# livesense-inc/fanlin-rs

Hardware: AMD Instinct MI355X
Metric: images/sec whole-node (1080p→300×200 resize+encode); p50 per-image ms (higher is better)
Workload: dtype u8 (exact, as f16 subnormals) x the reference's f32 weights as three f16 terms -> f32 sums (vertical, v_mfma_f32_16x16x32_f16); 24-bit fixed-point intermediate (2^-14 steps, three i8 planes) x 24-bit fixed-point weights (2^-24 steps, three i8 digits), eight of the nine digit products -> exact i32 (h

## Files before the change

fanlin-rs_amd/csrc/fl_batch.cpp:

```cpp
#include <stdio.h>
#include <stdlib.h>

#include <algorithm>
#include <cassert>
#include <memory>
#include <optional>

#include "fl_context.h"

using namespace fl;

namespace {


enum Stage1Kind { S1_NONE = 0, S1_PLACE = 1, S1_GENERIC = 2, S1_STREAM = 3, S1_NEAREST = 4, S1_MFMA = 5, S1_TILE = 6, S1_WTILE = 7 };
constexpr size_t kNoScratch = ~(size_t)0;

struct Work {
    flgpu_plan plan;
    const flgpu_params *p;
    uint32_t cs, pre, sw, sh;
    Stage1Kind s1;
    const uint8_t *src;
    uint8_t *s1_dst = nullptr;
// ... 156 lines not shown
                        const auto &v = by_job[jobs_in_order[r * T + t]];
                        for (uint32_t s2 = 0; s2 < S; ++s2) per_wg[triples[t][s2]].push_back(v[s2]);
                    }
                const uint32_t Lp = P - R * T;
                if (Lp) {
                    const uint32_t nt = (uint32_t)plan->tiles.size();
                    const uint32_t nb = std::max(1u, std::min(nt, (2u * G + Lp * S - 1u) / (Lp * S)));
                    const std::vector<MfmaItem> &bands = plan->items_for(nb);
                    std::vector<MfmaItem> units;
                    for (uint32_t p2 = R * T; p2 < P; ++p2)
                        for (MfmaItem u : bands) { u.job = jobs_in_order[p2]; units.push_back(u); }
                    std::stable_sort(units.begin(), units.end(), [](const MfmaItem &x, const MfmaItem &y) { return x.kb1 - x.kb0 > y.kb1 - y.kb0; });
                    std::vector<uint64_t> load(G, 0);
                    for (uint32_t b = 0; b < G; ++b) for (const MfmaItem &a : per_wg[b]) load[b] += a.kb1 - a.kb0;
                    for (const MfmaItem &u : units) {
                        uint32_t best = 0;
                        for (uint32_t b = 1; b < G; ++b) if (load[b] < load[best]) best = b;
                        per_wg[best].push_back(u);
                        load[best] += u.kb1 - u.kb0 + 2u;
                    }
                }
            }
        }
    }
    if (!uniform) { for (auto &v : per_wg) v.clear(); classic(); }
    std::vector<MfmaItem> flat;
    lists.assign(2u * G, 0u);
    for (uint32_t b = 0; b < G; ++b) {
        lists[2 * b] = (uint32_t)flat.size();
        lists[2 * b + 1] = (uint32_t)per_wg[b].size();
        flat.insert(flat.end(), per_wg[b].begin(), per_wg[b].end());
    }
    mitems.resize(base);
    mitems.insert(mitems.end(), flat.begin(), flat.end());
    nitems = (uint32_t)flat.size();
}

void fill_job(const Work &w, Job &j)
{
    memset(&j, 0, sizeof(j));
    const flgpu_plan &pl = w.plan;
    j.src = w.src;
    j.dst = w.s1_dst;
    j.src_bytes = w.sw * w.sh * w.cs;
    j.sw = w.sw; j.sh = w.sh;
    j.rw = pl.resized_w; j.rh = pl.resized_h;
    j.cx = pl.crop_x; j.cy = pl.crop_y;
    if (pl.letterboxed) {
        j.cw = std::min(pl.resized_w - pl.crop_x, pl.out_w - pl.place_x);
        j.ch = std::min(pl.resized_h - pl.crop_y, pl.out_h - pl.place_y);
    } else {
        j.cw = pl.out_w; j.ch = pl.out_h;
    }
    j.dw = pl.out_w; j.dh = pl.out_h;
    j.ox = pl.place_x; j.oy = pl.place_y;
    if (w.luma_mid) { j.dw = j.cw; j.dh = j.ch; j.ox = 0; j.oy = 0; }
    j.fill = (uint32_t)w.p->fill_r | ((uint32_t)w.p->fill_g << 8) | ((uint32_t)w.p->fill_b << 16) | (255u << 24);
    j.vtab = w.vtab; j.htab = w.htab;
    j.pad1 = w.tile_w;
    j.pad0 = w.tile_vplan;
    if (w.s1 == S1_NEAREST) {
        const float ry = (float)w.sh / (float)pl.resized_h, rx = (float)w.sw / (float)pl.resized_w;
        memcpy(&j.vtab, &ry, 4); memcpy(&j.htab, &rx, 4);
    }
}


uint32_t tile_width_for(const HostAxis &h, const HostAxis &v, uint32_t cx, uint32_t cw, uint32_t cy, uint32_t ch, uint32_t mc)
{
    for (uint32_t y0 = cy; y0 < cy + ch; y0 += 8u) {
        const uint32_t y1 = std::min(y0 + 8u, cy + ch);
        if (v.left[y1 - 1] + v.count[y1 - 1] - v.left[y0] > kTileVRows) return 0;
    }
    const uint32_t nc_max = kTileLdsFloats / (8u * mc);
    for (uint32_t tw = 256; tw >= 16; tw >>= 1) {
        bool fits = true;
        for (uint32_t x0 = cx; x0 < cx + cw && fits; x0 += tw) {
            const uint32_t x1 = std::min(x0 + tw, cx + cw);
            if (h.left[x1 - 1] + h.count[x1 - 1] - h.left[x0] > nc_max) fits = false;
            if (h.woff[x1 - 1] + h.count[x1 - 1] - h.woff[x0] > kTileWeightFloats) fits = false;
        }
        if (fits) return tw;
    }
    return 0;
}

void build_tile_vplan(const HostAxis &v, uint32_t cy, uint32_t ch, std::vector<uint32_t> &blk)
{
    const uint32_t nb = (ch + 7u) / 8u;
    uint32_t stride = 1;
    for (uint32_t b = 0; b < nb; ++b) {
        const uint32_t y0 = cy + 8u * b, y1 = std::min(y0 + 8u, cy + ch);
        stride = std::max(stride, v.left[y1 - 1] + v.count[y1 - 1] - v.left[y0]);
    }
    TileVPlanHeader hd{nb, stride, (uint32_t)(sizeof(TileVPlanHeader) / 4), (uint32_t)(sizeof(TileVPlanHeader) / 4) + 2u * nb};
    blk.assign((size_t)hd.dense_off + (size_t)nb * stride * 8u, 0u);
    memcpy(blk.data(), &hd, sizeof(hd));
    for (uint32_t b = 0; b < nb; ++b) {
        const uint32_t y0 = cy + 8u * b, y1 = std::min(y0 + 8u, cy + ch);
        const uint32_t top = v.left[y0], rv = v.left[y1 - 1] + v.count[y1 - 1] - top;
        blk[hd.bands_off + 2u * b] = top;
        blk[hd.bands_off + 2u * b + 1u] = rv;
        float *dense = reinterpret_cast<float *>(blk.data() + hd.dense_off) + (size_t)b * stride * 8u;
        for (uint32_t oy = y0; oy < y1; ++oy)
            for (uint32_t k = 0; k < v.count[oy]; ++k) dense[(size_t)(v.left[oy] + k - top) * 8u + (oy - y0)] = v.weights[v.woff[oy] + k];
    }
}

template <class Item, class Len>
void xcd_interleave(Item *first, uint32_t nitems, Len len_of)
{
#ifdef FL_EXPERIMENT
    static const bool no_xcd_order = [] { const char *e = getenv("FLGPU_NO_XCD_ORDER"); return e && e[0] == '1'; }();
#else
    constexpr bool no_xcd_order = false;
#endif
    std::vector<Item> tmp;
    for (uint32_t a = 0; a < nitems && !no_xcd_order;) {
        uint32_t b = a;
        const uint32_t len = len_of(first[a]);
        while (b < nitems && len_of(first[b]) == len) ++b;
        for (uint32_t g0 = a; g0 < b;) {
            uint32_t g1 = g0, njob = 0, prev = 0xffffffffu, per = 0, cur = 0;
            bool uniform = true;
            while (g1 < b) {
                if (first[g1].job != prev) {
                    if (njob == 8) break;
                    if (njob >= 1) { if (per == 0) per = cur; else if (cur != per) uniform = false; }
                    ++njob; prev = first[g1].job; cur = 0;
                }
                ++cur; ++g1;
            }
            if (per == 0) per = cur; else if (cur != per) uniform = false;
            if (uniform && njob > 1 && per > 1) {
                tmp.assign(first + g0, first + g1);
                for (uint32_t s2 = 0; s2 < per; ++s2)
                    for (uint32_t j2 = 0; j2 < njob; ++j2) first[g0 + s2 * njob + j2] = tmp[j2 * per + s2];
            }
            g0 = g1;
        }
        a = b;
    }
}



int jpeg_scratch(const flgpu_plan &pl, ScratchSizes &s)
{
    if (pl.out_w > 65535u || pl.out_h > 65535u) return FLGPU_ERR_UNSUPPORTED;
    const size_t units = (size_t)(pl.plane_w / 8u) * (pl.plane_h / 8u) * 3u;
    if (units * kJpegMaxUnitBytes * 8 >= ((size_t)1 << 32)) return FLGPU_ERR_UNSUPPORTED;
    s.jpeg_coef += align_up(units * sizeof(uint32_t), 256);
    s.jpeg_off += align_up((units + 1) * sizeof(uint32_t), 256);
    s.jpeg_raw += align_up(units * kAcWordsPerUnit * sizeof(uint32_t), 256);
    return FLGPU_OK;
}

int png_scratch(const flgpu_plan &pl, ScratchSizes &s)
{
    const uint64_t fb = png_filtered_bytes(pl.out_w, pl.out_h, pl.out_c);
    if ((uint64_t)s.png_rows + pl.out_h >= (1ull << 31) || (uint64_t)s.png_segs + png_segments(fb) >= (1ull << 31)) return FLGPU_ERR_UNSUPPORTED;
    s.png_filt += align_up(fb, 256);
    s.png_rows += pl.out_h;
    s.png_segs += (uint32_t)png_segments(fb);
    return FLGPU_OK;
}

int webpll_scratch(const flgpu_plan &pl, ScratchSizes &s)
{
    const uint64_t npix = (uint64_t)pl.out_w * pl.out_h;
    if ((uint64_t)s.wll_tiles + webpll_tiles(npix) >= (1ull << 31) || webpll_max_out_bytes(pl.out_w, pl.out_h) / 4u >= (1ull << 32))
        return FLGPU_ERR_UNSUPPORTED;
    s.wll_res += align_up(npix * 4u, 256);
    s.wll_tok += align_up(npix * 2u, 256);
    s.wll_stream += align_up(webpll_max_out_bytes(pl.out_w, pl.out_h), 256);
    s.wll_tiles += (uint32_t)webpll_tiles(npix);
    s.wll_pics++;
    return FLGPU_OK;
}

int plan_pictures(Batch &B, const flgpu_image *srcs, const flgpu_params *ps, bool same_params)
{
    for (size_t i = 0; i < B.n; ++i) {
        Work &w = B.work[i];
        const flgpu_image &s = srcs[i];
        w.p = same_params ? &ps[0] : &ps[i];
        if (!s.data || !B.dsts[i].data) return FLGPU_ERR_INVALID_ARG;
        int rc = flgpu_plan_output(w.p, s.width, s.height, s.channels, &w.plan);
        if (rc) return rc;
        if (s.capacity < (uint64_t)s.width * s.height * s.channels) return FLGPU_ERR_INVALID_ARG;
        if (B.dsts[i].capacity < w.plan.out_bytes) return FLGPU_ERR_BUFFER_TOO_SMALL;
        w.cs = s.channels; w.sw = w.plan.src_w; w.sh = w.plan.src_h;
        w.raw_w = s.width; w.raw_h = s.height;
        w.orient = w.p->orientation >= 2 ? w.p->orientation : 0;
        if (w.orient) { w.orient_off = B.scratch.o; B.scratch.o += align_up((size_t)s.width * s.height * s.channels, 256); }
        w.pre = w.p->grayscale ? PRE_GRAY : (w.p->inverse ? PRE_INVERT : PRE_NONE);
        w.src = s.data;
        w.final_dst = B.dsts[i].data;
        const flgpu_plan &pl = w.plan;
        const bool cropped = pl.crop_x || pl.crop_y || pl.out_w != pl.resized_w || pl.out_h != pl.resized_h;
        const bool pre_changes = (w.pre == PRE_INVERT) || (w.pre == PRE_GRAY && w.cs >= 3);
        if (!pre_changes) w.pre = PRE_NONE;
        if (pl.resampled) w.s1 = w.p->filter == FLGPU_FILTER_NEAREST ? S1_NEAREST : S1_GENERIC;
        else if (pre_changes || pl.letterboxed || cropped) w.s1 = S1_PLACE;
        else w.s1 = S1_NONE;
        const bool mfma_candidate = !B.dbg.on(DBG_NO_MFMA) && !B.dbg.on(DBG_FORCE_GENERIC) && (size_t)w.sw * w.cs >= 64u && (uint64_t)w.sh >= 2u * (uint64_t)pl.resized_h;
        if (pl.resampled && w.s1 == S1_GENERIC && !pre_changes && !w.orient && mfma_candidate && ((size_t)w.sw * w.cs) % 16u == 0 && (uintptr_t)s.data % 16u != 0) {
            w.align_off = B.scratch.al;
            B.scratch.al += align_up((size_t)s.width * s.height * s.channels, 256);
        }
        const bool blur = w.p->blur_sigma > 0.0f;
        const bool fe = w.p->front_end != FLGPU_FE_NONE;
        if (w.s1 != S1_NONE && !blur && !fe) w.s1_dst = w.final_dst;
        else if (w.s1 != S1_NONE) { w.s1_off = B.scratch.a; B.scratch.a += align_up(pl.pixel_bytes, 256); }
        if (blur && !fe) w.blur_dst = w.final_dst;
        else if (blur) { w.blur_off = B.scratch.b; B.scratch.b += align_up(pl.pixel_bytes, 256); }
        if (w.p->front_end == FLGPU_FE_JPEG) rc = jpeg_scratch(pl, B.scratch);
        if (w.p->front_end == FLGPU_FE_PNG) rc = png_scratch(pl, B.scratch);
        if (w.p->front_end == FLGPU_FE_WEBP_LOSSLESS) rc = webpll_scratch(pl, B.scratch);
        if (rc) return rc;
    }
    return FLGPU_OK;
}

int reserve_scratch(flgpu_ctx *c, Batch &B, hipStream_t st)
{
    const ScratchSizes &sz = B.scratch;
    FL_HIP(c, c->d_jpeg_coef.reserve(sz.jpeg_coef), "JPEG coefficient scratch");
    FL_HIP(c, c->d_jpeg_off.reserve(sz.jpeg_off), "JPEG offset scratch");
    FL_HIP(c, c->d_jpeg_raw.reserve(sz.jpeg_raw), "JPEG bit-stream scratch");
    FL_HIP(c, c->d_png_filt.reserve(sz.png_filt), "PNG filtered-row scratch");
    FL_HIP(c, c->d_png_chunks.reserve((size_t)sz.png_segs * kPngSegOutBytes), "PNG chunk scratch");
    FL_HIP(c, c->d_png_syms.reserve((size_t)sz.png_segs * kPngSegBytes * sizeof(uint16_t)), "PNG symbol scratch");
    FL_HIP(c, c->d_png_recs.reserve((size_t)sz.png_segs * 4u * sizeof(uint32_t)), "PNG segment records");
    FL_HIP(c, c->d_webpll_res.reserve(sz.wll_res), "WebP residual scratch");
    FL_HIP(c, c->d_webpll_tok.reserve(sz.wll_tok), "WebP token scratch");
    FL_HIP(c, c->d_webpll_tiles.reserve((size_t)sz.wll_tiles * sizeof(WebpllTile)), "WebP tile records");
    FL_HIP(c, c->d_webpll_pic.reserve((size_t)sz.wll_pics * kWebpllPicWords * sizeof(uint32_t)), "WebP per-picture scratch");
    FL_HIP(c, c->d_webpll_stream.reserve(sz.wll_stream), "WebP bit-stream scratch");
    FL_HIP(c, c->d_tmp_o.reserve(sz.o), "orientation scratch");
    FL_HIP(c, c->d_tmp_al.reserve(sz.al), "alignment scratch");
    for (auto &w : B.work)
        if (w.align_off != kNoScratch) {
            uint8_t *al = static_cast<uint8_t *>(c->d_tmp_al.p) + w.align_off;
            FL_HIP(c, hipMemcpyAsync(al, w.src, (size_t)w.sw * w.sh * w.cs, hipMemcpyDeviceToDevice, st), "alignment copy");
            w.src = al;
        }
    FL_HIP(c, c->d_tmp_a.reserve(sz.a), "scratch A");
    FL_HIP(c, c->d_tmp_b.reserve(sz.b), "scratch B");
    for (auto &w : B.work) {
        if (w.orient) { w.raw_src = w.src; w.src = static_cast<uint8_t *>(c->d_tmp_o.p) + w.orient_off; }
        if (w.s1 == S1_NONE) w.s1_dst = const_cast<uint8_t *>(w.src);
        if (w.s1_off != kNoScratch) w.s1_dst = static_cast<uint8_t *>(c->d_tmp_a.p) + w.s1_off;
        if (w.blur_off != kNoScratch) w.blur_dst = static_cast<uint8_t *>(c->d_tmp_b.p) + w.blur_off;
    }
    return FLGPU_OK;
}


bool arena_nearly_full(const flgpu_ctx *c) { return c->h_arena.size() >= c->arena_cap_words - 1024; }

template <class Map, class Build> uint32_t cached_block(flgpu_ctx *c, Map &cache, const typename Map::key_type &key, Build &&build)
{
    auto it = cache.find(key);
    if (it != cache.end()) return it->second;
    std::vector<uint32_t> blk;
    build(blk);
    const uint32_t off = arena_append(c, blk.data(), blk.size());
    if (off) cache.emplace(key, off);
    return off;
}

bool try_wtile(flgpu_ctx *c, Work &w, const Job &j)
{
    WtPlan *wp = get_wtile_plan(c, w.vk, *w.va, w.hk, *w.ha, j.cx, j.cy, j.cw, j.ch, w.cs);
    if (wp->arena_full || arena_nearly_full(c)) return false;
    if (wp->ok) { w.s1 = S1_WTILE; w.wplan = wp; }
    return true;
}

bool try_mfma(flgpu_ctx *c, const DebugSwitches &dbg, size_t n_resample, Work &w, const Job &j)
{
    MfmaPlan *mp = get_mfma_plan(c, w.vk, *w.va, w.hk, *w.ha, j.cx, j.cy, j.cw, j.ch, w.cs, dbg.on(DBG_MFMA_ARITH) ? MFMA_ARITH_PACKED : MFMA_ARITH_FULL);
    if (mp->arena_full || arena_nearly_full(c)) return false;
    if (!mp->ok) return true;
    uint32_t nbands = (uint32_t)std::max<int64_t>(0, dbg.get(DBG_FORCE_BANDS));
    if (!nbands && n_resample < 128) {
        const uint64_t G = std::max(1u, c->cu_count);
        uint64_t best = ~0ull;
        for (uint32_t b = 1; b <= std::min<uint32_t>(16u, (uint32_t)mp->tiles.size()); ++b) {
            const std::vector<MfmaItem> &cand = mp->items_for(b);
            uint32_t longest = 0;
            for (const MfmaItem &mi : cand) longest = std::max(longest, mi.kb1 - mi.kb0);
            const uint64_t cost = (((uint64_t)n_resample * cand.size() + G - 1) / G) * (longest + 2u);
            if (cost < best) { best = cost; nbands = b; }
        }
    }
    w.s1 = S1_MFMA; w.mplan = mp; w.mitems = &mp->items_for(std::max(nbands, 1u));
    return true;
}

bool try_stream(flgpu_ctx *c, const DebugSwitches &dbg, size_t n_resample, Work &w, const Job &j)
{
    uint32_t nbands = (uint32_t)std::max<int64_t>(0, dbg.get(DBG_FORCE_BANDS));
    if (!nbands && n_resample < 512) nbands = std::min((uint32_t)((1024 + n_resample * 2 - 1) / (n_resample * 2)), j.ch / 24u);
    nbands = std::min(std::max(nbands, 1u), std::max(1u, j.ch));
    const StreamPlan *sp = get_stream_plan(c, w.vk, *w.va, w.hk, *w.ha, j.cx, j.cy, j.cw, j.ch, nbands, w.cs, w.pre);
// ... 984 lines not shown
```

fanlin-rs_amd/csrc/fl_jpeg.h:

```cpp
#pragma once
#include <hip/hip_runtime.h>
#include <stdint.h>

namespace fl {

#define FL_JPEG_RESULT_OVERFLOW 4u
constexpr uint32_t kAcWordsPerUnit = 52;
struct alignas(16) JpegJob {
    const uint8_t *src;
    uint8_t *dst;
    uint32_t *meta;
    uint32_t *unit_off;
    uint32_t *acbits;
    uint32_t *result;
    uint32_t w, h, c;
    uint32_t bx, by;
    uint32_t tab_off;
    uint32_t pad0;
    uint32_t dst_cap;
};

hipError_t launch_jpeg_encode(const JpegJob *jobs, const uint32_t *arena, uint32_t job_base, uint32_t njobs, uint32_t max_blocks,
                              hipStream_t st);

}
```

fanlin-rs_amd/csrc/fl_jpeg.hip:

```cpp
#include <hip/hip_runtime.h>
#include <stdint.h>

#include "fl_jpeg.h"
#include "fl_jpeg_tables.h"
#include "fl_pixel.h"
#include "fl_types.h"

namespace fl {

namespace {


constexpr int32_t F_0_298 = 2446, F_0_390 = 3196, F_0_541 = 4433, F_0_765 = 6270, F_0_899 = 7373, F_1_175 = 9633, F_1_501 = 12299,
                  F_1_847 = 15137, F_1_961 = 16069, F_2_053 = 16819, F_2_562 = 20995, F_3_072 = 25172;

struct Mat8 { int32_t a[8][8]; };

constexpr void fdct_linear(const int32_t in[8], int32_t out[8])
{
    int32_t t0 = in[0] + in[7], t1 = in[1] + in[6], t2 = in[2] + in[5], t3 = in[3] + in[4];
    const int32_t t10 = t0 + t3, t11 = t1 + t2;
    int32_t t12 = t0 - t3, t13 = t1 - t2;
    t0 = in[0] - in[7]; t1 = in[1] - in[6]; t2 = in[2] - in[5]; t3 = in[3] - in[4];
    out[0] = t10 + t11;
    out[4] = t10 - t11;
    int32_t z1 = (t12 + t13) * F_0_541;
    out[2] = z1 + t12 * F_0_765;
    out[6] = z1 - t13 * F_1_847;
    t12 = t0 + t2;
    t13 = t1 + t3;
    z1 = (t12 + t13) * F_1_175;
    t12 = t12 * (-F_0_390) + z1;
    t13 = t13 * (-F_1_961) + z1;
    z1 = (t0 + t3) * (-F_0_899);
    out[1] = t0 * F_1_501 + z1 + t12;
    out[7] = t3 * F_0_298 + z1 + t13;
    z1 = (t1 + t2) * (-F_2_562);
    out[3] = t1 * F_3_072 + z1 + t13;
    out[5] = t2 * F_2_053 + z1 + t12;
}

constexpr Mat8 make_fdct_matrix()
{
    Mat8 m{};
    for (int j = 0; j < 8; ++j) {
        int32_t e[8] = {0, 0, 0, 0, 0, 0, 0, 0}, o[8] = {0, 0, 0, 0, 0, 0, 0, 0};
        e[j] = 1;
        fdct_linear(e, o);
        for (int k = 0; k < 8; ++k) m.a[k][j] = o[k];
    }
    return m;
}

__constant__ Mat8 kFdct = make_fdct_matrix();

constexpr bool fdct_matrix_fits_i16()
{
    const Mat8 m = make_fdct_matrix();
    for (int k = 0; k < 8; ++k)
        for (int j = 0; j < 8; ++j)
            if (m.a[k][j] > 32767 || m.a[k][j] < -32768) return false;
    return true;
}
static_assert(fdct_matrix_fits_i16(), "the passes use v_dot2_i32_i16: matrix entries must be 16-bit");

typedef short i16x2 __attribute__((ext_vector_type(2)));
__device__ __forceinline__ i16x2 as_i16x2(uint32_t v) { return __builtin_bit_cast(i16x2, v); }
__device__ __forceinline__ uint32_t pack_i16(int32_t lo, int32_t hi) { return ((uint32_t)lo & 0xffffu) | ((uint32_t)hi << 16); }
__device__ __forceinline__ int32_t dot8_i16(const uint32_t m[4], const uint4 v)
{
    int32_t p = __builtin_amdgcn_sdot2(as_i16x2(m[0]), as_i16x2(v.x), 0, false);
    p = __builtin_amdgcn_sdot2(as_i16x2(m[1]), as_i16x2(v.y), p, false);
    p = __builtin_amdgcn_sdot2(as_i16x2(m[2]), as_i16x2(v.z), p, false);
    return __builtin_amdgcn_sdot2(as_i16x2(m[3]), as_i16x2(v.w), p, false);
}

struct NaturalOrder { uint8_t n[64]; };
constexpr NaturalOrder make_natural()
{
    NaturalOrder t{};
    for (int k = 0; k < 64; ++k) t.n[k] = kUnzigzag[k];
    return t;
}
__constant__ NaturalOrder kNatural = make_natural();

struct HuffLut { uint32_t e[256]; };

constexpr HuffLut make_lut(const HuffSpec &s)
{
    HuffLut t{};
    uint32_t code = 0;
    int k = 0;
    for (int l = 1; l <= 16; ++l) {
        for (int i = 0; i < s.len[l - 1]; ++i, ++k) t.e[s.val[k]] = ((uint32_t)l << 16) | code++;
        code <<= 1;
    }
    return t;
}

struct HuffAll { HuffLut ac[2], dc[2]; };
constexpr HuffAll make_all() { return HuffAll{{make_lut(kAcLuma), make_lut(kAcChroma)}, {make_lut(kDcLuma), make_lut(kDcChroma)}}; }
__constant__ HuffAll kHuff = make_all();


template <int N>
__device__ __forceinline__ uint32_t dpp_row_shr(uint32_t v)
{
    return (uint32_t)__builtin_amdgcn_update_dpp(0, (int)v, 0x110 + N, 0xf, 0xf, false);
}

__device__ __forceinline__ uint32_t wave_inclusive_scan(uint32_t v, uint32_t lane)
{
    (void)lane;
    v += dpp_row_shr<1>(v);
    v += dpp_row_shr<2>(v);
    v += dpp_row_shr<4>(v);
    v += dpp_row_shr<8>(v);
    v += (uint32_t)__builtin_amdgcn_update_dpp(0, (int)v, 0x142, 0xa, 0xf, false);
    v += (uint32_t)__builtin_amdgcn_update_dpp(0, (int)v, 0x143, 0xc, 0xf, false);
    return v;
}

__device__ __forceinline__ void wave_lds_sync()
{
    __builtin_amdgcn_fence(__ATOMIC_SEQ_CST, "wavefront");
    __builtin_amdgcn_wave_barrier();
}

constexpr uint32_t kPackThreads = 512;
constexpr uint32_t kPackWaves = kPackThreads / 64;

__device__ __forceinline__ uint32_t wg_exclusive_scan(uint32_t v, uint32_t *s_w, uint32_t *total)
{
    const uint32_t lane = threadIdx.x & 63u, wave = threadIdx.x >> 6;
    const uint32_t inc = wave_inclusive_scan(v, lane);
    __syncthreads();
    if (lane == 63u) s_w[wave] = inc;
    __syncthreads();
    uint32_t base = 0, sum = 0;
#pragma unroll
    for (uint32_t i = 0; i < kPackWaves; ++i) { const uint32_t t = s_w[i]; if (i < wave) base += t; sum += t; }
    *total = sum;
    return base + inc - v;
}

__device__ __forceinline__ uint32_t coef_size(int32_t v)
{
    const uint32_t mag = (uint32_t)(v < 0 ? -v : v);
    return mag ? 32u - (uint32_t)__clz(mag) : 0u;
}


#ifndef FL_JPEG_BPW
#define FL_JPEG_BPW 16
#define FL_JPEG_WPG 2
#define FL_JPEG_PREFETCH 3
#endif
constexpr uint32_t kBlocksPerWave = FL_JPEG_BPW;
constexpr uint32_t kWavesPerWg = FL_JPEG_WPG;
constexpr uint32_t kPrefetch = FL_JPEG_PREFETCH;
static_assert(kBlocksPerWave == 32u || kBlocksPerWave == 16u, "the coding phase's lane mapping");
constexpr uint32_t kJpegThreads = 64u * kWavesPerWg;
constexpr uint32_t kBlocksPerWg = kWavesPerWg * kBlocksPerWave;
constexpr uint32_t kUnitsPerWave = 3u * kBlocksPerWave;

static_assert(63u * (16u + 10u) <= kAcWordsPerUnit * 32u, "a unit's AC code must fit its acbits slot");

struct WaveLds {
    int16_t coef[kUnitsPerWave][64];
    uint64_t nz[kUnitsPerWave];
    __attribute__((aligned(16))) int16_t smp[3][64];
    __attribute__((aligned(16))) int16_t p1[3][64];
};

__device__ __forceinline__ void stage_ac_luts(uint32_t *s_ac)
{
    for (uint32_t i = threadIdx.x; i < 512u; i += kJpegThreads) s_ac[i] = kHuff.ac[i >> 8].e[i & 255u];
    __syncthreads();
}

template <bool kRgba>
__device__ __forceinline__ uint32_t block_pixel(const JpegJob &jb, uint32_t brow, uint32_t bcol, uint32_t r, uint32_t c)
{
    uint32_t px = bcol * 8u + c, py = brow * 8u + r;
    px = px < jb.w ? px : jb.w - 1u;
    py = py < jb.h ? py : jb.h - 1u;
    if constexpr (kRgba) return ((const __attribute__((address_space(1))) uint32_t *)jb.src)[(size_t)py * jb.w + px];
    uint32_t pr, pg, pb, pa;
    load_rgba(jb.src + ((size_t)py * jb.w + px) * jb.c, jb.c, pr, pg, pb, pa);
    return pr | (pg << 8) | (pb << 16);
}

__device__ __forceinline__ void dct_quant_block(const uint32_t (&smp)[3], uint32_t nat, uint32_t r, uint32_t c, const uint32_t (&m1)[4],
                                                const uint32_t (&m2)[4], uint4 k1, const uint32_t (&q)[3], const uint32_t (&magic)[3],
                                                WaveLds &w, int32_t (&qv)[3])
{
#pragma unroll
    for (int k = 0; k < 3; ++k) w.smp[k][nat] = (int16_t)smp[k];
    wave_lds_sync();
#pragma unroll
    for (int k = 0; k < 3; ++k) {
        const int32_t p = dot8_i16(m1, *reinterpret_cast<const uint4 *>(w.smp[k] + r * 8));
        const int32_t v1 = ((p << k1.x) + (int32_t)k1.y) >> 11;
        w.p1[k][c * 8 + r] = (int16_t)v1;
    }
    wave_lds_sync();
#pragma unroll
    for (int k = 0; k < 3; ++k) {
        const int32_t p2 = dot8_i16(m2, *reinterpret_cast<const uint4 *>(w.p1[k] + c * 8));
        const int32_t d = (p2 + (int32_t)k1.z) >> k1.w;
        const int32_t sg = d >> 31;
        const uint32_t an = (uint32_t)((d ^ sg) - sg) >> 3;
        const uint32_t rq = __umulhi(2u * an + q[k], magic[k]);
        qv[k] = ((int32_t)rq ^ sg) - sg;
    }
}

typedef __attribute__((address_space(1))) uint32_t global_u32;

struct UnitBits {
    uint64_t acc;
    uint32_t pend, total, wi;
    global_u32 *out;
    __device__ __forceinline__ void put(uint32_t code, uint32_t len)
    {
        acc = (acc << len) | code;
        pend += len;
        total += len;
        if (pend >= 32u) { pend -= 32u; out[wi++] = (uint32_t)(acc >> pend); }
    }
};

template <bool kRgba>
__device__ __forceinline__ void transform_blocks(const JpegJob &jb, const uint32_t *__restrict__ arena, uint32_t first, uint32_t count,
                                                 uint32_t lane, WaveLds &w)
{
    const uint32_t nat = kNatural.n[lane], r = nat >> 3, c = nat & 7u;
    uint32_t m1[4], m2[4];
#pragma unroll
    for (int j = 0; j < 4; ++j) {
        m1[j] = pack_i16(kFdct.a[c][2 * j], kFdct.a[c][2 * j + 1]);
        m2[j] = pack_i16(kFdct.a[r][2 * j], kFdct.a[r][2 * j + 1]);
    }
    const uint8_t *qt = reinterpret_cast<const uint8_t *>(arena + jb.tab_off) + 624;
    const uint32_t *mg = reinterpret_cast<const uint32_t *>(qt + 128);
    const uint32_t q[3] = {qt[nat], qt[64 + nat], qt[64 + nat]};
    const uint32_t magic[3] = {mg[nat], mg[64 + nat], mg[64 + nat]};
    const uint4 k1 = {(c == 0u || c == 4u) ? 13u : 0u, c == 0u ? (uint32_t)(-(8 * 128) * 8192) : (c == 4u ? 0u : 1u << 10),
                      (r == 0u || r == 4u) ? 2u : 1u << 14, (r == 0u || r == 4u) ? 2u : 15u};
    uint32_t brow = first / jb.bx, bcol = first - brow * jb.bx;
    uint32_t ahead[kPrefetch];
#pragma unroll
    for (uint32_t j = 0; j < kPrefetch; ++j) {
        ahead[j] = block_pixel<kRgba>(jb, brow, bcol, r, c);
        if (++bcol == jb.bx) { bcol = 0; ++brow; }
    }
    for (uint32_t i = 0; i < count; ++i) {
        const uint32_t rgb = kRgba ? ahead[0] & 0xffffffu : ahead[0];
#pragma unroll
        for (uint32_t j = 0; j + 1u < kPrefetch; ++j) ahead[j] = ahead[j + 1u];
        ahead[kPrefetch - 1u] = block_pixel<kRgba>(jb, brow, bcol, r, c);
        if (++bcol == jb.bx) { bcol = 0; ++brow; }
        uint32_t smp[3];
        jfif_px(rgb, smp[0], smp[1], smp[2]);
        const bool flat = __ballot(rgb != (uint32_t)__builtin_amdgcn_readfirstlane((int)rgb)) == 0ull;
        if (flat) {
            if (lane == 0u) {
#pragma unroll
                for (int k = 0; k < 3; ++k) {
                    const int32_t d = 64 * ((int32_t)smp[k] - 128);
                    const int32_t sg = d >> 31;
                    const uint32_t an = (uint32_t)((d ^ sg) - sg) >> 3;
                    const uint32_t rq = __umulhi(2u * an + q[k], magic[k]);
                    w.coef[i * 3u + k][0] = (int16_t)(((int32_t)rq ^ sg) - sg);
                    w.nz[i * 3u + k] = 0ull;
                }
            }
            continue;
        }
        int32_t qv[3];
        dct_quant_block(smp, nat, r, c, m1, m2, k1, q, magic, w, qv);
#pragma unroll
        for (int k = 0; k < 3; ++k) {
            w.coef[i * 3u + k][lane] = (int16_t)qv[k];
            const uint64_t nz = __ballot(qv[k] != 0) & ~1ull;
            if (lane == 0u) w.nz[i * 3u + k] = nz;
        }
    }
}

__global__ __launch_bounds__(kJpegThreads) void jpeg_dct_quant_kernel(const JpegJob *__restrict__ jobs, const uint32_t *__restrict__ arena,
                                                                      uint32_t job_base)
{
    __shared__ WaveLds s_w[kWavesPerWg];
    __shared__ uint32_t s_ac[512];
    const JpegJob jb = jobs[job_base + blockIdx.y];
    const uint32_t wave = threadIdx.x >> 6, lane = threadIdx.x & 63u;
    const uint32_t nblocks = jb.bx * jb.by;
    if (blockIdx.x * kBlocksPerWg >= nblocks) return;
    stage_ac_luts(s_ac);
    const uint32_t first = blockIdx.x * kBlocksPerWg + wave * kBlocksPerWave;
    if (first >= nblocks) return;
    const uint32_t count = min(kBlocksPerWave, nblocks - first);
    WaveLds &w = s_w[wave];

    if (jb.c == 4u && (reinterpret_cast<uintptr_t>(jb.src) & 3u) == 0u) transform_blocks<true>(jb, arena, first, count, lane, w);
    else transform_blocks<false>(jb, arena, first, count, lane, w);
    wave_lds_sync();

    uint32_t b, u, u_end;
    bool chroma;
    if constexpr (kBlocksPerWave == 32u) {
        b = lane & 31u;
        chroma = lane >= 32u;
        u = b * 3u + (chroma ? 1u : 0u);
        u_end = b * 3u + (chroma ? 3u : 1u);
    } else {
        b = lane & 15u;
        chroma = lane >= 16u;
        u = b * 3u + (lane >> 4);
        u_end = lane >= 48u ? u : u + 1u;
    }
    if (b >= count) return;
    const uint32_t *tab = s_ac + (chroma ? 256u : 0u);
    const uint32_t eob = tab[0], zrl = tab[0xF0];
    for (; u < u_end; ++u) {
        const uint32_t unit = first * 3u + u;
        const int16_t *cf = w.coef[u];
        uint64_t m = w.nz[u];
        UnitBits ub{0ull, 0u, 0u, unit * kAcWordsPerUnit, (global_u32 *)jb.acbits};
        uint32_t prev = 0;
        uint32_t pos = (uint32_t)__builtin_ctzll(m | (1ull << 63));
        int32_t v = cf[pos];
        while (m) {
            const uint32_t cpos = pos;
            const int32_t cv = v;
            m &= m - 1ull;
            pos = (uint32_t)__builtin_ctzll(m | (1ull << 63));
            v = cf[pos];
            uint32_t run = cpos - prev - 1u;
            prev = cpos;
            while (run > 15u) { ub.put(zrl & 0xffffu, zrl >> 16); run -= 16u; }
            const uint32_t mag = (uint32_t)(cv < 0 ? -cv : cv);
            const uint32_t size = 32u - (uint32_t)__clz(mag);
            const uint32_t value = (uint32_t)(cv + (cv >> 31)) & ((1u << size) - 1u);
            const uint32_t e = tab[(run << 4) | size];
            ub.put(((e & 0xffffu) << size) | value, (e >> 16) + size);
        }
        if (prev != 63u) ub.put(eob & 0xffffu, eob >> 16);
        if (ub.pend) ub.out[ub.wi] = (uint32_t)(ub.acc << (32u - ub.pend));
        jb.meta[unit] = ((uint32_t)(uint16_t)cf[0]) | (ub.total << 16);
    }
}


constexpr uint32_t kWinWords = 8192;

__device__ __forceinline__ void win_or(uint32_t *win, uint32_t wbase, uint64_t g, uint32_t val)
{
    const uint64_t W = g >> 5;
    const uint32_t sh = (uint32_t)g & 31u;
    const uint32_t hi = val >> sh, lo = sh ? val << (32u - sh) : 0u;
    if (hi && W >= wbase && W < (uint64_t)wbase + kWinWords) atomicOr(&win[W - wbase], hi);
    if (lo && W + 1 >= wbase && W + 1 < (uint64_t)wbase + kWinWords) atomicOr(&win[W + 1 - wbase], lo);
}

__device__ __forceinline__ uint32_t dc_code(const JpegJob &jb, uint32_t u, uint32_t meta, uint32_t *len)
{
    const int32_t dc = (int16_t)(meta & 0xffffu), prev = u >= 3u ? (int32_t)(int16_t)(jb.meta[u - 3u] & 0xffffu) : 0;
    const int32_t diff = dc - prev;
    const uint32_t size = coef_size(diff);
    const uint32_t value = (uint32_t)(diff < 0 ? diff - 1 : diff) & ((1u << size) - 1u);
    const uint32_t e = kHuff.dc[(u % 3u) ? 1 : 0].e[size];
    *len = (e >> 16) + size;
    return (((e & 0xffffu) << size) | value) << (32u - *len);
}

__global__ __launch_bounds__(kPackThreads) void jpeg_pack_kernel(const JpegJob *__restrict__ jobs, const uint32_t *__restrict__ arena,
                                                                 uint32_t job_base)
{
    __shared__ uint32_t s_win[kWinWords];
    __shared__ uint32_t s_w[kPackWaves], s_carry, s_lo, s_hi;
    const JpegJob jb = jobs[job_base + blockIdx.x];
    const uint32_t tid = threadIdx.x;
    const uint32_t nunits = jb.bx * jb.by * 3u;
    constexpr uint32_t T = kPackThreads;

    for (uint32_t i = tid; i < kWinWords; i += T) s_win[i] = 0u;
    if (tid == 0u) s_carry = 0u;
    __syncthreads();
    for (uint32_t base = 0; base < nunits; base += T) {
        const uint32_t u = base + tid;
        uint32_t len = 0, dl = 0, dcw = 0, nw = 0, a0 = 0, a1 = 0;
        if (u < nunits) {
            const uint32_t m = jb.meta[u];
            nw = ((m >> 16) + 31u) >> 5;
            if (nw > 0u) a0 = jb.acbits[(size_t)u * kAcWordsPerUnit];
            if (nw > 1u) a1 = jb.acbits[(size_t)u * kAcWordsPerUnit + 1u];
            dcw = dc_code(jb, u, m, &dl);
            len = dl + (m >> 16);
        }
        uint32_t chunk;
        const uint32_t ex = wg_exclusive_scan(len, s_w, &chunk);
        const uint32_t carry = s_carry;
        if (u < nunits) {
            const uint32_t off = carry + ex;
            jb.unit_off[u] = off;
            win_or(s_win, 0u, off, dcw);
            if (nw > 0u) win_or(s_win, 0u, (uint64_t)off + dl, a0);
            if (nw > 1u) win_or(s_win, 0u, (uint64_t)off + dl + 32u, a1);
            for (uint32_t w = 2; w < nw; ++w) win_or(s_win, 0u, (uint64_t)off + dl + 32u * w, jb.acbits[(size_t)u * kAcWordsPerUnit + w]);
        }
        __syncthreads();
        if (tid == 0u) s_carry = carry + chunk;
        __syncthreads();
    }
    const uint32_t total_bits = s_carry;
    if (tid == 0u) jb.unit_off[nunits] = total_bits;
    __threadfence_block();
    __syncthreads();
    const uint32_t nbytes = (total_bits + 7u) >> 3, limit = jb.dst_cap;
    const uint8_t *hdr = reinterpret_cast<const uint8_t *>(arena + jb.tab_off);
    for (uint32_t i = tid; i < kJpegHeaderBytes; i += T) if (i < limit) jb.dst[i] = hdr[i];

    uint32_t ff_before = 0;
    for (uint32_t wbase = 0; wbase * 32ull < total_bits; wbase += kWinWords) {
        const uint64_t wb = (uint64_t)wbase * 32u, we = wb + (uint64_t)kWinWords * 32u;
        if (wbase != 0u) {
            for (uint32_t i = tid; i < kWinWords; i += T) s_win[i] = 0u;
            if (tid == 0u) {
                uint32_t lo = 0, hi = nunits;
                while (lo < hi) { const uint32_t mid = (lo + hi) >> 1; if (jb.unit_off[mid + 1u] > wb) hi = mid; else lo = mid + 1u; }
                s_lo = lo;
                uint32_t lo2 = lo, hi2 = nunits;
                while (lo2 < hi2) { const uint32_t mid = (lo2 + hi2) >> 1; if (jb.unit_off[mid] >= we) hi2 = mid; else lo2 = mid + 1u; }
                s_hi = lo2;
            }
        } else if (tid == 0u) { s_lo = 0u; s_hi = 0u; }
        __syncthreads();
        const uint32_t u_lo = s_lo, u_hi = s_hi;
        for (uint32_t ub = u_lo; ub < u_hi; ub += T / 2u) {
            const uint32_t u = ub + (tid >> 1), j = tid & 1u;
            if (u < u_hi) {
                const uint32_t m = jb.meta[u], off = jb.unit_off[u];
                uint32_t dl;
                const uint32_t dcw = dc_code(jb, u, m, &dl);
                if (j == 0u) win_or(s_win, wbase, off, dcw);
                const uint32_t nw = ((m >> 16) + 31u) >> 5;
                for (uint32_t w = j; w < nw; w += 2u)
                    win_or(s_win, wbase, (uint64_t)off + dl + 32u * w, jb.acbits[(size_t)u * kAcWordsPerUnit + w]);
            }
        }
        __syncthreads();
        if (tid == 0u && (total_bits & 7u) && (total_bits >> 5) >= wbase && (total_bits >> 5) < wbase + kWinWords)
            s_win[(total_bits >> 5) - wbase] |= (0xFFu >> (total_bits & 7u)) << (24u - 8u * ((total_bits >> 3) & 3u));
        __syncthreads();
        const uint32_t win_bytes = (uint32_t)min((uint64_t)kWinWords * 4u, (uint64_t)nbytes - (uint64_t)wbase * 4u);
        if (tid == 0u) s_carry = 0u;
        __syncthreads();
        for (uint32_t base = 0; base < win_bytes; base += 4u * T) {
            const uint32_t i = base + tid * 4u;
            const uint32_t word = i < win_bytes ? s_win[i >> 2] : 0u;
            const uint32_t valid = i < win_bytes ? (win_bytes - i < 4u ? win_bytes - i : 4u) : 0u;
            uint32_t ff = 0;
#pragma unroll
            for (uint32_t k = 0; k < 4; ++k) ff += (k < valid && ((word >> (24u - 8u * k)) & 255u) == 255u) ? 1u : 0u;
            uint32_t chunk;
            const uint32_t ex = wg_exclusive_scan(ff, s_w, &chunk);
            const uint32_t carry = s_carry;
            uint64_t o = (uint64_t)kJpegHeaderBytes + (uint64_t)wbase * 4u + i + ff_before + carry + ex;
#pragma unroll
            for (uint32_t k = 0; k < 4; ++k) {
                if (k < valid) {
                    const uint32_t b = (word >> (24u - 8u * k)) & 255u;
                    if (o < limit) jb.dst[o] = (uint8_t)b;
                    ++o;
                    if (b == 255u) { if (o < limit) jb.dst[o] = 0u; ++o; }
                }
            }
            __syncthreads();
            if (tid == 0u) s_carry = carry + chunk;
            __syncthreads();
        }
        ff_before += s_carry;
        __syncthreads();
    }
    if (tid == 0u) {
        const uint64_t end = (uint64_t)kJpegHeaderBytes + nbytes + ff_before;
        if (end + 2u <= limit) {
            jb.dst[end] = 0xFF; jb.dst[end + 1u] = 0xD9;
            jb.result[1] = (uint32_t)(end + 2u);
        } else {
            jb.result[1] = 0u;
            atomicOr(&jb.result[0], FL_JPEG_RESULT_OVERFLOW);
        }
    }
}

}

hipError_t launch_jpeg_encode(const JpegJob *jobs, const uint32_t *arena, uint32_t job_base, uint32_t njobs, uint32_t max_blocks,
                              hipStream_t st)
{
    if (!njobs || !max_blocks) return hipSuccess;
    hipLaunchKernelGGL(jpeg_dct_quant_kernel, dim3((max_blocks + kBlocksPerWg - 1) / kBlocksPerWg, njobs), dim3(kJpegThreads), 0, st, jobs, arena, job_base);
    FL_LAUNCH_CHECK();
    hipLaunchKernelGGL(jpeg_pack_kernel, dim3(njobs), dim3(kPackThreads), 0, st, jobs, arena, job_base);
    FL_LAUNCH_CHECK();
    return hipSuccess;
}

}
```

Measured before the change: 539,500.

## Interleave JPEG AC scratch by unit groups and trim pack-kernel barriers

The per-unit AC bitstream scratch now uses an interleaved layout: each group of 48 units stores word w of every unit contiguously, so reads across neighbouring units coalesce. The pack kernel drops the shared carry variable. It keeps the running totals in registers from the scan totals and double-buffers the scan's per-wave partials, which cuts several __syncthreads per iteration down to one LDS-only barrier. It also prefetches the next iteration's meta and first AC words, keeps the DC Huffman table in LDS, and clears the window with vector stores. The risks are subtle barrier-correctness problems in the reduced synchronisation, and that the writes from the coding phase become strided.

```diff
diff --git a/fanlin-rs_amd/csrc/fl_batch.cpp b/fanlin-rs_amd/csrc/fl_batch.cpp
--- a/fanlin-rs_amd/csrc/fl_batch.cpp
+++ b/fanlin-rs_amd/csrc/fl_batch.cpp
@@ -332,7 +332,7 @@
     if (units * kJpegMaxUnitBytes * 8 >= ((size_t)1 << 32)) return FLGPU_ERR_UNSUPPORTED;
     s.jpeg_coef += align_up(units * sizeof(uint32_t), 256);
     s.jpeg_off += align_up((units + 1) * sizeof(uint32_t), 256);
-    s.jpeg_raw += align_up(units * kAcWordsPerUnit * sizeof(uint32_t), 256);
+    s.jpeg_raw += align_up(ac_scratch_words(units) * sizeof(uint32_t), 256);
     return FLGPU_OK;
 }
 
diff --git a/fanlin-rs_amd/csrc/fl_jpeg.h b/fanlin-rs_amd/csrc/fl_jpeg.h
--- a/fanlin-rs_amd/csrc/fl_jpeg.h
+++ b/fanlin-rs_amd/csrc/fl_jpeg.h
@@ -6,6 +6,27 @@
 
 #define FL_JPEG_RESULT_OVERFLOW 4u
 constexpr uint32_t kAcWordsPerUnit = 52;
+constexpr uint32_t kAcGroupUnits = 48;
+__host__ __device__ constexpr uint32_t ac_word_index(uint32_t u, uint32_t w)
+{
+    return (u / kAcGroupUnits) * (kAcGroupUnits * kAcWordsPerUnit) + w * kAcGroupUnits + u % kAcGroupUnits;
+}
+__host__ __device__ constexpr size_t ac_scratch_words(size_t units)
+{
+    return (units + kAcGroupUnits - 1) / kAcGroupUnits * kAcGroupUnits * kAcWordsPerUnit;
+}
+constexpr bool ac_index_is_injective()
+{
+    bool seen[kAcGroupUnits * kAcWordsPerUnit] = {};
+    for (uint32_t u = 0; u < kAcGroupUnits; ++u)
+        for (uint32_t w = 0; w < kAcWordsPerUnit; ++w) {
+            const uint32_t i = ac_word_index(u, w);
+            if (i >= kAcGroupUnits * kAcWordsPerUnit || seen[i]) return false;
+            seen[i] = true;
+        }
+    return ac_word_index(kAcGroupUnits, 0) == kAcGroupUnits * kAcWordsPerUnit;
+}
+static_assert(ac_index_is_injective(), "every (unit, word) of a group has its own word of the group's slot");
 struct alignas(16) JpegJob {
     const uint8_t *src;
     uint8_t *dst;
diff --git a/fanlin-rs_amd/csrc/fl_jpeg.hip b/fanlin-rs_amd/csrc/fl_jpeg.hip
--- a/fanlin-rs_amd/csrc/fl_jpeg.hip
+++ b/fanlin-rs_amd/csrc/fl_jpeg.hip
@@ -103,6 +103,8 @@
 __constant__ HuffAll kHuff = make_all();
 
 
+typedef __attribute__((address_space(1))) uint32_t global_u32;
+
 template <int N>
 __device__ __forceinline__ uint32_t dpp_row_shr(uint32_t v)
 {
@@ -127,6 +129,13 @@
     __builtin_amdgcn_wave_barrier();
 }
 
+__device__ __forceinline__ void lds_barrier()
+{
+    __builtin_amdgcn_fence(__ATOMIC_RELEASE, "workgroup", "local");
+    __builtin_amdgcn_s_barrier();
+    __builtin_amdgcn_fence(__ATOMIC_ACQUIRE, "workgroup", "local");
+}
+
 constexpr uint32_t kPackThreads = 512;
 constexpr uint32_t kPackWaves = kPackThreads / 64;
 
@@ -134,9 +143,8 @@
 {
     const uint32_t lane = threadIdx.x & 63u, wave = threadIdx.x >> 6;
     const uint32_t inc = wave_inclusive_scan(v, lane);
-    __syncthreads();
     if (lane == 63u) s_w[wave] = inc;
-    __syncthreads();
+    lds_barrier();
     uint32_t base = 0, sum = 0;
 #pragma unroll
     for (uint32_t i = 0; i < kPackWaves; ++i) { const uint32_t t = s_w[i]; if (i < wave) base += t; sum += t; }
@@ -163,6 +171,7 @@
 constexpr uint32_t kJpegThreads = 64u * kWavesPerWg;
 constexpr uint32_t kBlocksPerWg = kWavesPerWg * kBlocksPerWave;
 constexpr uint32_t kUnitsPerWave = 3u * kBlocksPerWave;
+static_assert(kUnitsPerWave % kAcGroupUnits == 0u, "a wave codes whole groups of the AC scratch");
 
 static_assert(63u * (16u + 10u) <= kAcWordsPerUnit * 32u, "a unit's AC code must fit its acbits slot");
 
@@ -215,8 +224,6 @@
         qv[k] = ((int32_t)rq ^ sg) - sg;
     }
 }
-
-typedef __attribute__((address_space(1))) uint32_t global_u32;
 
 struct UnitBits {
     uint64_t acc;
@@ -227,7 +234,7 @@
         acc = (acc << len) | code;
         pend += len;
         total += len;
-        if (pend >= 32u) { pend -= 32u; out[wi++] = (uint32_t)(acc >> pend); }
+        if (pend >= 32u) { pend -= 32u; out[wi] = (uint32_t)(acc >> pend); wi += kAcGroupUnits; }
     }
 };
 
@@ -328,7 +335,7 @@
         const uint32_t unit = first * 3u + u;
         const int16_t *cf = w.coef[u];
         uint64_t m = w.nz[u];
-        UnitBits ub{0ull, 0u, 0u, unit * kAcWordsPerUnit, (global_u32 *)jb.acbits};
+        UnitBits ub{0ull, 0u, 0u, 0u, (global_u32 *)jb.acbits + ac_word_index(unit, 0u)};
         uint32_t prev = 0;
         uint32_t pos = (uint32_t)__builtin_ctzll(m | (1ull << 63));
         int32_t v = cf[pos];
@@ -365,58 +372,71 @@
     if (lo && W + 1 >= wbase && W + 1 < (uint64_t)wbase + kWinWords) atomicOr(&win[W + 1 - wbase], lo);
 }
 
-__device__ __forceinline__ uint32_t dc_code(const JpegJob &jb, uint32_t u, uint32_t meta, uint32_t *len)
-{
-    const int32_t dc = (int16_t)(meta & 0xffffu), prev = u >= 3u ? (int32_t)(int16_t)(jb.meta[u - 3u] & 0xffffu) : 0;
+__device__ __forceinline__ uint32_t dc_code(const uint32_t *s_dc, uint32_t u, uint32_t meta, uint32_t meta_prev, uint32_t *len)
+{
+    const int32_t dc = (int16_t)(meta & 0xffffu), prev = u >= 3u ? (int32_t)(int16_t)(meta_prev & 0xffffu) : 0;
     const int32_t diff = dc - prev;
     const uint32_t size = coef_size(diff);
     const uint32_t value = (uint32_t)(diff < 0 ? diff - 1 : diff) & ((1u << size) - 1u);
-    const uint32_t e = kHuff.dc[(u % 3u) ? 1 : 0].e[size];
+    const uint32_t e = s_dc[((u % 3u) ? 16u : 0u) + size];
     *len = (e >> 16) + size;
     return (((e & 0xffffu) << size) | value) << (32u - *len);
 }
 
+struct PackUnit { uint32_t m, mp, a0, a1; };
+__device__ __forceinline__ PackUnit load_pack_unit(const global_u32 *meta, const global_u32 *acbits, uint32_t u, uint32_t nunits)
+{
+    u = u < nunits ? u : nunits - 1u;
+    return PackUnit{meta[u], meta[u >= 3u ? u - 3u : 0u], acbits[ac_word_index(u, 0u)], acbits[ac_word_index(u, 1u)]};
+}
+
+__device__ __forceinline__ void clear_window(uint32_t *win)
+{
+    for (uint32_t i = threadIdx.x; i < kWinWords / 4u; i += kPackThreads) reinterpret_cast<uint4 *>(win)[i] = uint4{0u, 0u, 0u, 0u};
+}
+
 __global__ __launch_bounds__(kPackThreads) void jpeg_pack_kernel(const JpegJob *__restrict__ jobs, const uint32_t *__restrict__ arena,
                                                                  uint32_t job_base)
 {
-    __shared__ uint32_t s_win[kWinWords];
-    __shared__ uint32_t s_w[kPackWaves], s_carry, s_lo, s_hi;
+    __shared__ __attribute__((aligned(16))) uint32_t s_win[kWinWords];
+    __shared__ uint32_t s_w[2][kPackWaves], s_dc[32], s_lo, s_hi;
     const JpegJob jb = jobs[job_base + blockIdx.x];
+    const global_u32 *meta = (const global_u32 *)jb.meta, *acbits = (const global_u32 *)jb.acbits;
+    global_u32 *unit_off = (global_u32 *)jb.unit_off;
     const uint32_t tid = threadIdx.x;
     const uint32_t nunits = jb.bx * jb.by * 3u;
     constexpr uint32_t T = kPackThreads;
-
-    for (uint32_t i = tid; i < kWinWords; i += T) s_win[i] = 0u;
-    if (tid == 0u) s_carry = 0u;
+    uint32_t par = 0;
+
+    if (tid < 32u) s_dc[tid] = kHuff.dc[tid >> 4].e[tid & 15u];
+    PackUnit next = load_pack_unit(meta, acbits, tid, nunits);
+    clear_window(s_win);
     __syncthreads();
+    uint32_t total_bits = 0;
     for (uint32_t base = 0; base < nunits; base += T) {
         const uint32_t u = base + tid;
-        uint32_t len = 0, dl = 0, dcw = 0, nw = 0, a0 = 0, a1 = 0;
+        const PackUnit cur = next;
+        next = load_pack_unit(meta, acbits, u + T, nunits);
+        uint32_t len = 0, dl = 0, dcw = 0, nw = 0;
         if (u < nunits) {
-            const uint32_t m = jb.meta[u];
-            nw = ((m >> 16) + 31u) >> 5;
-            if (nw > 0u) a0 = jb.acbits[(size_t)u * kAcWordsPerUnit];
-            if (nw > 1u) a1 = jb.acbits[(size_t)u * kAcWordsPerUnit + 1u];
-            dcw = dc_code(jb, u, m, &dl);
-            len = dl + (m >> 16);
+            nw = ((cur.m >> 16) + 31u) >> 5;
+            dcw = dc_code(s_dc, u, cur.m, cur.mp, &dl);
+            len = dl + (cur.m >> 16);
         }
         uint32_t chunk;
-        const uint32_t ex = wg_exclusive_scan(len, s_w, &chunk);
-        const uint32_t carry = s_carry;
+        const uint32_t ex = wg_exclusive_scan(len, s_w[par], &chunk);
+        par ^= 1u;
         if (u < nunits) {
-            const uint32_t off = carry + ex;
-            jb.unit_off[u] = off;
+            const uint32_t off = total_bits + ex;
+            unit_off[u] = off;
             win_or(s_win, 0u, off, dcw);
-            if (nw > 0u) win_or(s_win, 0u, (uint64_t)off + dl, a0);
-            if (nw > 1u) win_or(s_win, 0u, (uint64_t)off + dl + 32u, a1);
-            for (uint32_t w = 2; w < nw; ++w) win_or(s_win, 0u, (uint64_t)off + dl + 32u * w, jb.acbits[(size_t)u * kAcWordsPerUnit + w]);
-        }
-        __syncthreads();
-        if (tid == 0u) s_carry = carry + chunk;
-        __syncthreads();
-    }
-    const uint32_t total_bits = s_carry;
-    if (tid == 0u) jb.unit_off[nunits] = total_bits;
+            if (nw > 0u) win_or(s_win, 0u, (uint64_t)off + dl, cur.a0);
+            if (nw > 1u) win_or(s_win, 0u, (uint64_t)off + dl + 32u, cur.a1);
+            for (uint32_t w = 2; w < nw; ++w) win_or(s_win, 0u, (uint64_t)off + dl + 32u * w, acbits[ac_word_index(u, w)]);
+        }
+        total_bits += chunk;
+    }
+    if (tid == 0u) unit_off[nunits] = total_bits;
     __threadfence_block();
     __syncthreads();
     const uint32_t nbytes = (total_bits + 7u) >> 3, limit = jb.dst_cap;
@@ -427,37 +447,33 @@
     for (uint32_t wbase = 0; wbase * 32ull < total_bits; wbase += kWinWords) {
         const uint64_t wb = (uint64_t)wbase * 32u, we = wb + (uint64_t)kWinWords * 32u;
         if (wbase != 0u) {
-            for (uint32_t i = tid; i < kWinWords; i += T) s_win[i] = 0u;
+            clear_window(s_win);
             if (tid == 0u) {
                 uint32_t lo = 0, hi = nunits;
-                while (lo < hi) { const uint32_t mid = (lo + hi) >> 1; if (jb.unit_off[mid + 1u] > wb) hi = mid; else lo = mid + 1u; }
+                while (lo < hi) { const uint32_t mid = (lo + hi) >> 1; if (unit_off[mid + 1u] > wb) hi = mid; else lo = mid + 1u; }
                 s_lo = lo;
                 uint32_t lo2 = lo, hi2 = nunits;
-                while (lo2 < hi2) { const uint32_t mid = (lo2 + hi2) >> 1; if (jb.unit_off[mid] >= we) hi2 = mid; else lo2 = mid + 1u; }
+                while (lo2 < hi2) { const uint32_t mid = (lo2 + hi2) >> 1; if (unit_off[mid] >= we) hi2 = mid; else lo2 = mid + 1u; }
                 s_hi = lo2;
             }
-        } else if (tid == 0u) { s_lo = 0u; s_hi = 0u; }
-        __syncthreads();
-        const uint32_t u_lo = s_lo, u_hi = s_hi;
-        for (uint32_t ub = u_lo; ub < u_hi; ub += T / 2u) {
-            const uint32_t u = ub + (tid >> 1), j = tid & 1u;
-            if (u < u_hi) {
-                const uint32_t m = jb.meta[u], off = jb.unit_off[u];
-                uint32_t dl;
-                const uint32_t dcw = dc_code(jb, u, m, &dl);
-                if (j == 0u) win_or(s_win, wbase, off, dcw);
-                const uint32_t nw = ((m >> 16) + 31u) >> 5;
-                for (uint32_t w = j; w < nw; w += 2u)
-                    win_or(s_win, wbase, (uint64_t)off + dl + 32u * w, jb.acbits[(size_t)u * kAcWordsPerUnit + w]);
+            __syncthreads();
+            const uint32_t u_lo = s_lo, u_hi = s_hi;
+            for (uint32_t ub = u_lo; ub < u_hi; ub += T / 2u) {
+                const uint32_t u = ub + (tid >> 1), j = tid & 1u;
+                if (u < u_hi) {
+                    const uint32_t m = meta[u], off = unit_off[u];
+                    uint32_t dl;
+                    const uint32_t dcw = dc_code(s_dc, u, m, meta[u >= 3u ? u - 3u : 0u], &dl);
+                    if (j == 0u) win_or(s_win, wbase, off, dcw);
+                    const uint32_t nw = ((m >> 16) + 31u) >> 5;
+                    for (uint32_t w = j; w < nw; w += 2u) win_or(s_win, wbase, (uint64_t)off + dl + 32u * w, acbits[ac_word_index(u, w)]);
+                }
             }
         }
-        __syncthreads();
         if (tid == 0u && (total_bits & 7u) && (total_bits >> 5) >= wbase && (total_bits >> 5) < wbase + kWinWords)
-            s_win[(total_bits >> 5) - wbase] |= (0xFFu >> (total_bits & 7u)) << (24u - 8u * ((total_bits >> 3) & 3u));
+            atomicOr(&s_win[(total_bits >> 5) - wbase], (0xFFu >> (total_bits & 7u)) << (24u - 8u * ((total_bits >> 3) & 3u)));
         __syncthreads();
         const uint32_t win_bytes = (uint32_t)min((uint64_t)kWinWords * 4u, (uint64_t)nbytes - (uint64_t)wbase * 4u);
-        if (tid == 0u) s_carry = 0u;
-        __syncthreads();
         for (uint32_t base = 0; base < win_bytes; base += 4u * T) {
             const uint32_t i = base + tid * 4u;
             const uint32_t word = i < win_bytes ? s_win[i >> 2] : 0u;
@@ -466,9 +482,9 @@
 #pragma unroll
             for (uint32_t k = 0; k < 4; ++k) ff += (k < valid && ((word >> (24u - 8u * k)) & 255u) == 255u) ? 1u : 0u;
             uint32_t chunk;
-            const uint32_t ex = wg_exclusive_scan(ff, s_w, &chunk);
-            const uint32_t carry = s_carry;
-            uint64_t o = (uint64_t)kJpegHeaderBytes + (uint64_t)wbase * 4u + i + ff_before + carry + ex;
+            const uint32_t ex = wg_exclusive_scan(ff, s_w[par], &chunk);
+            par ^= 1u;
+            uint64_t o = (uint64_t)kJpegHeaderBytes + (uint64_t)wbase * 4u + i + ff_before + ex;
 #pragma unroll
             for (uint32_t k = 0; k < 4; ++k) {
                 if (k < valid) {
@@ -478,12 +494,8 @@
                     if (b == 255u) { if (o < limit) jb.dst[o] = 0u; ++o; }
                 }
             }
-            __syncthreads();
-            if (tid == 0u) s_carry = carry + chunk;
-            __syncthreads();
-        }
-        ff_before += s_carry;
-        __syncthreads();
+            ff_before += chunk;
+        }
     }
     if (tid == 0u) {
         const uint64_t end = (uint64_t)kJpegHeaderBytes + nbytes + ff_before;
```

Result: faster. 561,600 (median of 6 runs) (+4.1%).
